# thelovelab/DESeq2

Measured on AMD Instinct MI355X. Metric: genes/sec for DESeq() disp+beta+Wald fit, 50k x 500 x p=4 (throughput of steps pipelined two deep; one call at a time: one_call_at_a_time), higher is better.
Workload: dtype f64; 1 GPU; BASELINE configs[2]: 50k genes x 500 samples, ~batch+condition (p=4), Wald; 50000 non-zero genes in total, sharded over 1 GPU(s) in the contiguous ranges of R/parallel.R:10; inputs resident in HBM in R layout (int32 counts, f64 nf matrix; the fused chain reads the size factors as the m-vector the matrix was built from); genes_total=50000, genes_this_gpu=50000, samples=500, p=4, test=Wald, parallelism=gene-shard x1, chain=fused device-driven (dsq_deseq_dev), steps_overlap=step k enqueued while step k-1's results are copied and post-processed

## Files before the change

### deseq2_amd/csrc/ctx.hip

```cpp
#include "../../include/deseq2_mi355x.h"
#include "dsq_internal.hpp"

#include <cstdarg>
#include <cstdio>
#include <cstdlib>
#include <cstring>
#include <map>
#include <memory>
#include <mutex>
#include <vector>

namespace dsq {

thread_local char g_err[512] = "";
std::mutex g_mu;

int capi_fail(int code, const char *fmt, ...) {
    va_list ap;
    va_start(ap, fmt);
    vsnprintf(g_err, sizeof g_err, fmt, ap);
    va_end(ap);
    return code;
}

int env_int(const char *name, int dflt) {
    const char *v = getenv(name);
    return (v && *v) ? atoi(v) : dflt;
}

const Tuning &tuning() {
    static Tuning t = {env_int("DSQ_BETA_WAVES", 4), env_int("DSQ_BETA_STAGE", -1), env_int("DSQ_BETA_BPC", 0),
                       env_int("DSQ_BETA_LDS_KB", 160),
                       env_int("DSQ_DISP_WAVES", 4), env_int("DSQ_DISP_STAGE", -1), env_int("DSQ_DISP_BPC", 0),
                       env_int("DSQ_DISP_LDS_KB", 160), env_int("DSQ_ABLATE", 0), env_int("DSQ_FORCE_ITERS", 0),
                       env_int("DSQ_DISP_XLDS", 1), env_int("DSQ_BETA_XLDS", 1), env_int("DSQ_DYNAMIC", 1),
                       env_int("DSQ_BETA_CELLS", 1), env_int("DSQ_DISP_CELL_MINP", DSQ_DISP_CELL_MINP),
                       env_int("DSQ_OVERLAP", 1), env_int("DSQ_LPT", 1),
                       env_int("DSQ_LPT_MAXN", 16384), env_int("DSQ_LPT_KEY2", 0)};
    return t;
}

int device_cu_count() {
    static int cached[kMaxDevices];
    int dev = 0;
    if (hipGetDevice(&dev) != hipSuccess || dev < 0 || dev >= kMaxDevices) return 256;
    if (cached[dev] == 0) {
        int v = 0;
        if (hipDeviceGetAttribute(&v, hipDeviceAttributeMultiprocessorCount, dev) != hipSuccess || v <= 0) v = 256;
        cached[dev] = v;
    }
    return cached[dev];
}

// ... 202 lines not shown
```

### deseq2_amd/csrc/dsq_internal.hpp

```cpp
#pragma once
#include <hip/hip_runtime.h>
#include <stdint.h>
#include <functional>
#include <mutex>
#include <string.h>

namespace dsq {

struct DispKernelParams {
    int n, m, p;
    long ld;
    const int32_t *y;
    const double *mu_hat;
    const double *weights;
    const double *x;
    const double *log_alpha_in;
    const double *prior_mean;
    double prior_sigmasq, min_log_alpha, kappa_0, tol, weightThreshold;
    int maxit, usePrior, useWeights, useCR;
    double *log_alpha;
    int32_t *iter, *iter_accept;
    double *last_change, *initial_lp, *initial_dlp, *last_lp, *last_dlp, *last_d2lp;
    const double *grid;
    int ngrid;
// ... 26 lines not shown
    int maxit, useQR, useWeights;
    double *beta_mat, *beta_var_mat, *iter, *hat_diagonals, *contrast_num, *contrast_denom, *deviance;
    double *mu_out;
    double *scratch;
    double *cscratch;
    int ablate, force_iters;
    int xlds;
    int *work_counter;
    const int32_t *rows;
    const int32_t *n_dev;
    int rows_few;
    const int32_t *cell_perm, *cell_start;
    int ncell;
    double *kconst_out;
    int p_true;
};

struct PrefitKernelParams {
    int n, m, p;
    long ld;
    const int32_t *y;
    const double *nf;
    int nf_is_vector;
    const double *weights;
    int useWeights;
    const double *q, *a, *r;
    double *baseMean, *baseVar, *roughDisp, *beta_init;
    int32_t *allZero;
    const int32_t *rows;
    const int32_t *n_dev;
// ... 56 lines not shown
struct CooksKernelParams {
    int n, m, p;
    long ld;
    const int32_t *y;
    const double *nf;
    int nf_is_vector;
    const double *mu, *H;
    const int32_t *perm;
    const int32_t *cell_start;
    const int32_t *in3;
    int ncell, any3;
    int sortcap;
    double *cooks, *maxCooks, *robustDisp;
    const int32_t *rows;
    const int32_t *n_dev;
};

struct ReplaceKernelParams {
    int n, m;
    long ld;
    const int32_t *y;
    const double *nf;
    int nf_is_vector;
    const double *cooks;
    double cutoff, trim;
    const int32_t *replaceable;
    int sortcap;
    int32_t *newCounts, *replace;
    const int32_t *rows;
    const int32_t *n_dev;
};

struct SizeFactorKernelParams {
    int n, m;
    const void *y;
    long y_si, y_sj;
    const double *nm;
    long nm_si, nm_sj;
    const double *geoMeans;
    const int32_t *control;
    int type;
    int stabilize;
    double *sf;
    double *lgm_out;
    double *nf_out;
// ... 113 lines not shown
template <int P> hipError_t launch_fit_beta_p(const BetaKernelParams &kp, hipStream_t st);
template <int P> hipError_t launch_optim_p(const OptimKernelParams &kp, hipStream_t st);
template <int P> void fit_beta_scratch_doubles(int n, int m, int use_weights, size_t *slab, size_t *cscr);

struct Tuning {
    int beta_waves, beta_stage, beta_bpc, beta_lds_kb;
    int disp_waves, disp_stage, disp_bpc, disp_lds_kb;
    int ablate, force_iters;
    int disp_xlds, beta_xlds;
    int dynamic;
    int beta_cells;
    int disp_cell_minp;
    int overlap;
    int lpt, lpt_maxn;
    int lpt_key2;
};
const Tuning &tuning();

hipError_t launch_transpose_r_to_gm_f64(const double *src, double *dst, int n, int m, long ld, hipStream_t st);
hipError_t launch_transpose_r_to_gm_i32(const int32_t *src, int32_t *dst, int n, int m, long ld, hipStream_t st);
hipError_t launch_counts_f64_to_gm_i32(const double *src, int32_t *dst, int n, int m, long ld, int32_t *bad, hipStream_t st);
hipError_t launch_transpose_gm_to_r_f64(const double *src, double *dst, int n, int m, long ld, hipStream_t st);
hipError_t launch_transpose_gm_to_r_i32(const int32_t *src, int32_t *dst, int n, int m, long ld, hipStream_t st);
hipError_t launch_test_math(int op, const double *a, const double *b, const double *c, double *out, long n, hipStream_t st);

constexpr int kMaxDevices = 64;
int device_cu_count();
#define DSQ_CACHE_PER_DEVICE(a, b)                                                        \
    do {                                                                                  \
        static thread_local int cache_dev_ = -1;                                          \
// ... 10 lines not shown
        if (e_ != hipSuccess)                                                                    \
            return capi_fail(e_ == hipErrorOutOfMemory ? DSQ_ERR_NOMEM : DSQ_ERR_DEVICE, "%s: %s", #expr, \
                             hipGetErrorString(e_));                                             \
    } while (0)
int env_int(const char *name, int dflt);
extern std::mutex g_mu;
void capi_latch_stream(hipStream_t s);
int capi_ws_get(int slot, size_t bytes, void **out);
int capi_upload_table(int slot, const void *src, size_t bytes, hipStream_t st, void **dev_out);
int capi_check_device();
int capi_upload_cells(const int32_t *labels, int m, int slot, hipStream_t st, const int32_t **perm_dev,
                      const int32_t **start_dev);
hipError_t launch_fit_beta_rolled(const BetaKernelParams &kp, hipStream_t st);
void fit_beta_rolled_scratch_doubles(int n, int m, int p, int useW, size_t *slab, size_t *cscr);
hipError_t dispatch_fit_beta(int p, const BetaKernelParams &kp, hipStream_t st, bool *ok);
void dispatch_beta_scratch(int p, int n, int m, int useW, size_t *slab, size_t *cscr);
hipError_t dispatch_fit_disp(int p, const DispKernelParams &kp, hipStream_t st, bool grid, bool *ok);
bool fit_disp_rolled_applies(const DispKernelParams &kp, int *p_true);
hipError_t dispatch_optim_rows(int p, const OptimKernelParams &kp, hipStream_t st, bool *ok);
void capi_prof_begin(const char *name, int n, hipStream_t st);
void capi_prof_end(hipStream_t st);
bool capi_prof_on();
int capi_side_stream(hipStream_t *side, hipEvent_t *fork_ev, hipEvent_t *join_ev);
int capi_host_sharded(size_t n, const std::function<int(size_t, size_t, hipStream_t, int, int)> &f, int max_shards);
int capi_host_shards(size_t n);
int stage_h2d(void *dev, const void *host, size_t e, size_t n_total, size_t lo, size_t cnt, size_t cols, hipStream_t st);
int stage_d2h(void *host, const void *dev, size_t e, size_t n_total, size_t lo, size_t cnt, size_t cols, hipStream_t st);
void stage_prefault(void *host, size_t bytes);
void stage_prefault_finish();
struct PrefaultScope { ~PrefaultScope() { stage_prefault_finish(); } };
// ... 7 lines not shown
```

### deseq2_amd/csrc/fit_beta.hip

```cpp
#ifndef DSQ_BETA_WIDE_MIN
#define DSQ_BETA_WIDE_MIN 10
#endif
#define DSQ_WIDE_MIN DSQ_BETA_WIDE_MIN
#include "dsq_internal.hpp"
#include <cstdio>
#include <cstdlib>
#include "dsq_math.hpp"
#include "dsq_wave.hpp"
#include "../../include/dsq_arith_spec.h"
#include "fit_beta_common.hpp"
#include "dsq_prof.hpp"

namespace dsq {

template <int P>
struct SymNB { static constexpr int value = P * (P + 1) / 2; };

#define DSQ_BETA_ARENA_MIN DSQ_WIDE_MIN
#if DSQ_P >= DSQ_BETA_ARENA_MIN
#define DSQ_BWORK(T, name) T &name = *reinterpret_cast<T *>(arena + arena_off); arena_off += (int)((sizeof(T) + 7) / 8)
#define DSQ_BMARK(name) const int name = arena_off
#define DSQ_BRESET(name) arena_off = name
#define DSQ_UNROLL_Q _Pragma("unroll")
#else
// ... 668 lines not shown
#endif

__host__ __device__ static inline size_t beta_cell_int_doubles(int m) { return (((size_t)DSQ_CMAX + 2 + m + 3) / 4) * 2; }
__host__ __device__ static inline size_t beta_cell_wave_doubles(int m, bool use_w) {
    (void)m; (void)use_w;
    return (4 + 16) * (size_t)DSQ_CMAX;
}
static_assert((4 + 16) * DSQ_CMAX >= kIrlsTab / 2 + 2 * kIrlsTab, "the constants pass borrows the wave's cell slab + park area");

#ifdef DSQ_WIDE_PROF
__device__ unsigned long long betac_prof[DSQ_PROF_SLOTS];
#define DSQ_CPROF(slot) do { const unsigned long long t1_ = clock64(); pacc_k[slot] += t1_ - pt0_k; pt0_k = t1_; } while (0)
#else
#define DSQ_CPROF(slot)
#endif
template <int P, bool USE_W>
__global__ void __launch_bounds__(256, DSQ_BETA_CELL_MINW) fit_beta_cell_kernel(BetaKernelParams kp) {
    extern __shared__ __attribute__((aligned(16))) double smem[];
    const int lane = threadIdx.x & 63;
    const int wave = threadIdx.x >> 6;
    const int waves = blockDim.x >> 6;
    const int m = kp.m;
    const int C = kp.ncell;
    const int Mrows = C + P;
    const int nwork = DSQ_NWORK(kp);
    if (blockIdx.x * waves >= nwork) return;
    double *xcs = smem;
    int32_t *starts = reinterpret_cast<int32_t *>(smem + (size_t)DSQ_CMAX * P);
    int32_t *pc = starts + DSQ_CMAX + 2;
    const size_t lnf_doubles = kp.nf_is_vector ? (size_t)m : 0;
// ... 322 lines not shown
                    for (int k = 1; k < P; k++) eta = __builtin_fma(xcs[cl * P + k], beta[k], eta);
                    double h = 0.0;
#pragma unroll
                    for (int i1 = 0; i1 < P; i1++) {
                        const double x1 = xcs[cl * P + i1];
#pragma unroll
                        for (int i2 = 0; i2 < P; i2++) h += x1 * (xcs[cl * P + i2] * lane_read(Gic[i2], i1));
                    }
                    if (lane < C) {
                        slab[4 * lane] = expl;
                        slab[4 * lane + 2] = dexp(eta);
                        slab[4 * lane + 3] = h;
                    }
                }
                wave_lds_sync();
                for (int k = lane; k < m; k += 64) {
                    const int pk = pc[k];
                    const int j = pk & 0x3ffffff, c = pk >> 26;
                    const double nf = nfg[j];
                    if (kp.hat_diagonals) {
                        const double mu = __builtin_fmax(nf * slab[4 * c], minmu);
                        const double rcp = 1.0 / (1.0 + alpha * mu);
                        double wv;
                        if constexpr (USE_W) wv = mu * (wg[j] * rcp);
                        else wv = mu * rcp;
                        kp.hat_diagonals[(size_t)g * kp.ld + j] = wv * slab[4 * c + 3];
                    }
                    if (kp.mu_out) {
                        double v = nf * slab[4 * c + 2];
                        if (kp.mu_floor > 0.0) v = __builtin_fmax(v, kp.mu_floor);
                        kp.mu_out[(size_t)g * kp.ld + j] = v;
                    }
                }
            }
            DSQ_CPROF(6);
            double Tc[P], Sgc[P];
            lane_mat_mul<P>(Gic, Gc, Tc);
            lane_mat_mul<P>(Tc, Gic, Sgc);
            double cn = 0.0;
#pragma unroll
            for (int c = 0; c < P; c++) cn = __builtin_fma(kp.contrast[c], beta[c], cn);
            double rr = 0.0;
#pragma unroll
            for (int a = 0; a < P; a++) rr = __builtin_fma(kp.contrast[a], Sgc[a], rr);
            double cd = 0.0;
#pragma unroll
            for (int b = 0; b < P; b++) cd = __builtin_fma(lane_read(rr, b), kp.contrast[b], cd);
// ... 36 lines not shown
            wave_lds_sync();
            if (lane < C) {
                double eta = xcs[lane * P] * beta[0];
#pragma unroll
                for (int k = 1; k < P; k++) eta = __builtin_fma(xcs[lane * P + k], beta[k], eta);
                double h = 0.0;
#pragma unroll
                for (int i1 = 0; i1 < P; i1++)
#pragma unroll
                    for (int i2 = 0; i2 < P; i2++) h += xcs[lane * P + i1] * (xcs[lane * P + i2] * Gi[i2][i1]);
                slab[4 * lane] = expl;
                slab[4 * lane + 2] = dexp(eta);
                slab[4 * lane + 3] = h;
            }
            wave_lds_sync();
            for (int k = lane; k < m; k += 64) {
                const int pk = pc[k];
                const int j = pk & 0x3ffffff, c = pk >> 26;
                const double nf = nfg[j];
                if (kp.hat_diagonals) {
                    const double mu = __builtin_fmax(nf * slab[4 * c], minmu);
                    const double rcp = 1.0 / (1.0 + alpha * mu);
                    double wv;
                    if constexpr (USE_W) wv = mu * (wg[j] * rcp);
                    else wv = mu * rcp;
                    kp.hat_diagonals[(size_t)g * kp.ld + j] = wv * slab[4 * c + 3];
                }
                if (kp.mu_out) {
                    double v = nf * slab[4 * c + 2];
                    if (kp.mu_floor > 0.0) v = __builtin_fmax(v, kp.mu_floor);
                    kp.mu_out[(size_t)g * kp.ld + j] = v;
                }
            }
        }
        DSQ_CPROF(6);
        double T[P][P], Sg[P][P];
        mat_mul<P>(Gi, G, T);
        mat_mul<P>(T, Gi, Sg);
        double cn = 0.0;
#pragma unroll
        for (int c = 0; c < P; c++) cn = __builtin_fma(contrast[c], beta[c], cn);
        double cd = 0.0;
#pragma unroll
        for (int b = 0; b < P; b++) {
            double rr = 0.0;
#pragma unroll
            for (int a = 0; a < P; a++) rr = __builtin_fma(contrast[a], Sg[a][b], rr);
// ... 377 lines not shown
#else
    int waves, grid, xlds;
    bool stage;
    size_t lds;
    beta_geometry<DSQ_P>(n, m, useW != 0, &waves, &stage, &xlds, &grid, &lds);
    *slab = stage ? 0 : (size_t)grid * waves * (size_t)m * kSlabVecs;
    *cscr = 0;
    if (DSQ_P >= rolled_minp()) {
        size_t s2 = 0, c2 = 0;
        fit_beta_rolled_scratch_doubles(n, m, DSQ_P, useW, &s2, &c2);
        if (s2 > *slab) *slab = s2;
    }
#endif
}

template <>
hipError_t launch_fit_beta_p<DSQ_P>(const BetaKernelParams &kp0, hipStream_t st) {
    if constexpr (DSQ_P <= DSQ_SPEC_BETA_CELL_MAXP)
        if (kp0.ncell > 0 && kp0.ncell <= DSQ_CMAX && kp0.ncell + DSQ_P <= 64) return launch_beta_cells<DSQ_P>(kp0, st);
#if DSQ_P >= DSQ_BETA_ROLLED_MIN
    return launch_fit_beta_rolled(kp0, st);
#else
    if (DSQ_P >= rolled_minp()) return launch_fit_beta_rolled(kp0, st);
    int waves, grid, xlds;
    bool stage;
    size_t lds;
    int qr = 0;
    beta_geometry<DSQ_P>(kp0.n, kp0.m, kp0.useWeights != 0, &waves, &stage, &xlds, &grid, &lds,
                         kp0.useQR != 0 && kp0.maxit > 0, &qr);
    BetaKernelParams kp = kp0;
    kp.xlds = xlds;
    if (kp.rows_few && grid > device_cu_count()) grid = device_cu_count();
    constexpr int kQr = (DSQ_P >= DSQ_BETA_QRROWS_MIN) ? 1 : 0, kQreg = (DSQ_P >= DSQ_BETA_QRREG_MIN) ? 2 : 0;
    constexpr int kQreg2 = (DSQ_P >= DSQ_BETA_QRREG_MIN && DSQ_P <= DSQ_BETA_QRREG2_MAXP) ? 3 : 0;
// ... 32 lines not shown
```

### deseq2_amd/csrc/outlier.hip

```cpp
#include "dsq_internal.hpp"
#include "dsq_math.hpp"
#include "dsq_wave.hpp"
#include <type_traits>

namespace dsq {

DSQ_DEV void wave_sort(double *b, int n2, int lane) {
    wave_lds_sync();
    for (int k = 2; k <= n2; k <<= 1) {
        for (int j = k >> 1; j > 0; j >>= 1) {
            for (int t = lane; t < (n2 >> 1); t += 64) {
                int lo = ((t & ~(j - 1)) << 1) | (t & (j - 1));
                int hi = lo | j;
                bool asc = (lo & k) == 0;
                double a = b[lo], c = b[hi];
                if ((a > c) == asc) { b[lo] = c; b[hi] = a; }
            }
            wave_lds_sync();
        }
    }
}

DSQ_DEV void wave_merge_bitonic(double *b, int n2, int lane) {
    wave_lds_sync();
// ... 35 lines not shown

static constexpr int kOutlierBatch = 4;

__global__ void __launch_bounds__(256) cooks_kernel(CooksKernelParams kp) {
    extern __shared__ double smem[];
    const int lane = threadIdx.x & 63;
    const int wave = threadIdx.x >> 6;
    const int waves = blockDim.x >> 6;
    const int m = kp.m;
    double *cn = smem + (size_t)wave * (m + kp.sortcap);
    double *buf = cn + m;
    const double inf = __builtin_inf();
    const int nwork = DSQ_NWORK(kp);
    for (int wi = blockIdx.x * waves + wave; wi < nwork; wi += gridDim.x * waves) {
        const int g = DSQ_GENE(kp, wi);
        const int32_t *yg = kp.y + (size_t)g * kp.ld;
        const double *nfg = kp.nf_is_vector ? kp.nf : kp.nf + (size_t)g * kp.ld;
        double acc = 0.0;
        {
            int32_t yb[kOutlierBatch];
            double nb[kOutlierBatch];
            sweep_batched<kOutlierBatch>(m, lane, [&](int j, int b) { yb[b] = yg[j]; nb[b] = nfg[j]; },
                                         [&](int j, int b) {
                                             const double v = (double)yb[b] / nb[b];
                                             cn[j] = v;
                                             acc += v;
                                         });
        }
        const double mean_all = wave_allreduce(acc) / (double)m;
        double v;
// ... 101 lines not shown
    }
}

__global__ void __launch_bounds__(256) replace_kernel(ReplaceKernelParams kp) {
    extern __shared__ double smem[];
    const int lane = threadIdx.x & 63;
    const int wave = threadIdx.x >> 6;
    const int waves = blockDim.x >> 6;
    const int m = kp.m;
    double *buf = smem + (size_t)wave * kp.sortcap;
    const double inf = __builtin_inf();
    const int n2 = pow2_at_least(m);
    const int nwork = DSQ_NWORK(kp);
    for (int wi = blockIdx.x * waves + wave; wi < nwork; wi += gridDim.x * waves) {
        const int g = DSQ_GENE(kp, wi);
        const int32_t *yg = kp.y + (size_t)g * kp.ld;
        const double *nfg = kp.nf_is_vector ? kp.nf : kp.nf + (size_t)g * kp.ld;
        const double *ckg = kp.cooks + (size_t)g * kp.ld;
        int any = 0;
        {
            double cb[kOutlierBatch];
            sweep_batched<kOutlierBatch>(m, lane, [&](int j, int b) { cb[b] = ckg[j]; },
                                         [&](int, int b) { if (cb[b] > kp.cutoff) any = 1; });
        }
        any = __any(any);
        int32_t *og = kp.newCounts + (size_t)g * kp.ld;
        if (!any) {
            int32_t yb[kOutlierBatch];
            sweep_batched<kOutlierBatch>(m, lane, [&](int j, int b) { yb[b] = yg[j]; }, [&](int j, int b) { og[j] = yb[b]; });
        } else {
// ... 19 lines not shown

template <typename KP, typename F>
static hipError_t launch_outlier(F fn, const KP &kp, size_t doubles_per_wave, hipStream_t st, bool *ok) {
    int waves = outlier_waves(doubles_per_wave);
    *ok = waves > 0;
    if (!*ok) return hipSuccess;
    size_t lds = (size_t)waves * doubles_per_wave * 8;
    if (lds > 64 * 1024) {
        hipError_t e = hipFuncSetAttribute((const void *)fn, hipFuncAttributeMaxDynamicSharedMemorySize, (int)lds);
        if (e != hipSuccess) return e;
    }
    int blocks = (kp.n + waves - 1) / waves;
    int per_cu = (int)((160 * 1024) / (lds ? lds : 1));
    if (per_cu > 8) per_cu = 8;
    if (per_cu < 1) per_cu = 1;
    int cap = device_cu_count() * per_cu;
    if (blocks > cap) blocks = cap;
    if (blocks < 1) blocks = 1;
    hipLaunchKernelGGL(fn, dim3(blocks), dim3(64 * waves), lds, st, kp);
    return hipGetLastError();
}

hipError_t launch_cooks(const CooksKernelParams &kp0, hipStream_t st, bool *ok) {
    CooksKernelParams kp = kp0;
    if (kp.sortcap < 64) kp.sortcap = 64;
    return launch_outlier(cooks_kernel, kp, (size_t)kp.m + kp.sortcap, st, ok);
}

hipError_t launch_replace(const ReplaceKernelParams &kp, hipStream_t st, bool *ok) {
    return launch_outlier(replace_kernel, kp, (size_t)kp.sortcap, st, ok);
}
// ... 3 lines not shown
```

### deseq2_amd/csrc/pipeline.hip

```cpp
#include "capi.hpp"
#include "dsq_math.hpp"
#include "dsq_wave.hpp"

#include <algorithm>
#include <cstdio>
#include <cstdlib>
#include <cstring>
#include <vector>

namespace dsq {

DSQ_DEV double np_min(double a, double b) { return (a != a || b != b) ? a + b : (a < b ? a : b); }
DSQ_DEV double np_max(double a, double b) { return (a != a || b != b) ? a + b : (a > b ? a : b); }

struct Rows {
    const int32_t *rows;
    const int32_t *n_dev;
    int n;
};
DSQ_DEV int rows_count(const Rows &r) { return r.n_dev ? *r.n_dev : r.n; }
DSQ_DEV int rows_gene(const Rows &r, int i) { return r.rows ? r.rows[i] : i; }

__global__ void __launch_bounds__(1024) compact_kernel(int mode, int n, int32_t *allZero, const int32_t *force_zero,
                                                       const double *mean_in, const double *disp_in, double thresh,
// ... 206 lines not shown
                const double z = q.beta[(size_t)g + (size_t)q.n * c] / q.betaSE[(size_t)g + (size_t)q.n * c];
                q.stat[(size_t)g + (size_t)q.n * c] = z;
                q.pvalue[(size_t)g + (size_t)q.n * c] = dpnorm_upper2(z);
            }
        }
    }
}

__global__ void list_kernel(Rows rw, const int32_t *flag, int want, int32_t *rows_out, int32_t *count) {
    const int i = blockIdx.x * blockDim.x + threadIdx.x;
    if (i >= rows_count(rw)) return;
    const int g = rows_gene(rw, i);
    if ((flag[g] != 0) == (want != 0)) rows_out[atomicAdd(count, 1)] = g;
}

struct NaRowsParams {
    Rows rw;
    int n, p;
    const int32_t *allZero, *n_refit;
    double *beta, *betaSE, *stat, *pvalue, *betaIter, *logLike, *logLikeReduced, *maxCooks;
    int32_t *betaConv;
};
__global__ void na_rows_kernel(NaRowsParams q) {
    const int i = blockIdx.x * blockDim.x + threadIdx.x;
    if (i >= rows_count(q.rw) || *q.n_refit <= 0) return;
    const int g = rows_gene(q.rw, i);
    if (!q.allZero[g]) return;
    const double nan = dnan();
    for (int c = 0; c < q.p; c++) {
        q.beta[(size_t)g + (size_t)q.n * c] = nan;
// ... 145 lines not shown
    const int32_t *red_cell_perm, *red_cell_start;
    int red_ncell;
    int32_t *cells_dev;
    void *trend_ws, *sel_ws;
    int pkp, pmax;
    int next_counter;
    const int32_t *cell_perm, *cell_start;
    int ncell;
    const char *tag;
    double t_tol, t_minmu, ge_floor;
    int t_maxit, t_useQR;
    hipStream_t side;
    hipEvent_t ev_fork, ev_join;
    bool overlap, forked, ll_pending;
    LogLikeKernelParams ll;
    int any3, maxcell, all_replaceable;
};

enum { CNT_NZ = DSQ_ST_N_NONZERO, CNT_GRID1 = DSQ_ST_N_GRID_GENEEST, CNT_TREND = DSQ_ST_N_TREND, CNT_GRID2 = DSQ_ST_N_GRID_MAP,
       CNT_OPT1 = DSQ_ST_N_OPTIM_GENEEST, CNT_OPT2 = DSQ_ST_N_OPTIM_TEST, CNT_REP = DSQ_ST_N_REPLACE, CNT_REFIT = DSQ_ST_N_REFIT,
       CNT_GRID1R = DSQ_ST_N_GRID_GENEEST_REFIT, CNT_GRID2R = DSQ_ST_N_GRID_MAP_REFIT, CNT_OPT1R = DSQ_ST_N_OPTIM_GENEEST_REFIT,
       CNT_OPT2R = DSQ_ST_N_OPTIM_TEST_REFIT, CNT_OPT3 = 14, CNT_OPT3R = 15, CNT_N = DSQ_ST_COUNT };
static_assert(DSQ_ST_N_OPTIM_TEST_REFIT < 14 && DSQ_ST_COUNT == 16, "status block layout");

static int *next_work_counter(Pipe &P) {
    int *c = P.work_counters + (P.next_counter % 60);
    P.next_counter++;
    return c;
}

// ... 43 lines not shown
    int ncell;
    int p_true;
};
static DesignSel design_of(const Pipe &P, int which) {
    const DsqDeseqArgs *a = P.a;
    DesignSel d;
    if (which == DES_REDUCED) d = {P.red_x_k, P.red_binit, P.red_lam, P.red_pk, P.red_cell_perm, P.red_cell_start, P.red_ncell, a->p_red};
    else if (which == DES_PRIOR) d = {P.pri_x_k, a->prior_expanded ? P.red_binit : P.beta_init, P.lam_prior, P.pri_pk,
                                      P.cell_perm, P.cell_start, P.ncell, a->p_prior};
    else d = {P.x_k, P.beta_init, P.lam, P.pk, P.cell_perm, P.cell_start, P.ncell, P.p};
    return d;
}

static int launch_fit_beta(Pipe &P, const Rows &rw, const int32_t *y, const double *alpha, const double *weights,
                           double *mu_out, double mu_floor, double *hat, double tol, int maxit, int useQR, double minmu,
                           const char *name, int which = DES_FULL) {
    const DesignSel ds = design_of(P, which);
    BetaKernelParams kp = fit_head<BetaKernelParams>(P, rw, y, weights);
    kp.p = ds.p; kp.x = ds.x; kp.alpha_hat = alpha; kp.contrast = P.contrast;
    kp.beta_init = ds.beta_init; kp.lambda = ds.lam;
    kp.tol = tol; kp.minmu = minmu; kp.mu_floor = mu_floor; kp.maxit = maxit; kp.useQR = useQR ? 1 : 0;
    kp.beta_mat = P.beta_nat; kp.beta_var_mat = P.beta_var; kp.iter = P.beta_iter;
    kp.contrast_num = P.cnum; kp.contrast_denom = P.cden; kp.deviance = P.dev;
    kp.hat_diagonals = hat; kp.mu_out = mu_out;
    kp.kconst_out = P.kconst;
    kp.scratch = P.scratch; kp.cscratch = P.cscratch;
    kp.work_counter = next_work_counter(P);
    kp.rows_few = rows_few(P, rw);
    kp.cell_perm = ds.cperm; kp.cell_start = ds.cstart; kp.ncell = ds.ncell;
    kp.p_true = ds.p_true;
    bool ok = false;
    char nm[32];
    snprintf(nm, sizeof nm, "%s%s", name, P.tag);
// ... 234 lines not shown
    DSQ_HIP(hipGetLastError());
    return DSQ_OK;
}

hipError_t launch_loglike_side(const LogLikeKernelParams &kp, hipStream_t st);
hipError_t launch_xim_flagged(const double *nf, int n, int m, long ld, const int32_t *want_a, const int32_t *want_b, double *scratch_m,
                              double *out, hipStream_t st);
static int join_side(Pipe &P) {
    if (!P.forked) return DSQ_OK;
    P.forked = false;
    DSQ_HIP(hipEventRecord(P.ev_join, P.side));
    DSQ_HIP(hipStreamWaitEvent(P.st, P.ev_join, 0));
    return DSQ_OK;
}

static int launch_pending_ll(Pipe &P, bool beside) {
    if (!P.ll_pending) return DSQ_OK;
    P.ll_pending = false;
    if (beside) {
        DSQ_HIP(hipEventRecord(P.ev_fork, P.st));
        DSQ_HIP(hipStreamWaitEvent(P.side, P.ev_fork, 0));
        DSQ_HIP(launch_loglike_side(P.ll, P.side));
        P.forked = true;
    } else {
        DSQ_HIP(launch_loglike(P.ll, P.st));
    }
    return DSQ_OK;
}

static int test_fit(Pipe &P, const Rows &rw, const int32_t *y, double *mu_out, double *hat, int cnt_optim) {
    const DsqDeseqArgs *a = P.a;
    const DsqDeseqOut *o = P.o;
    if (a->betaPrior) return mle_fit(P, rw, y, mu_out, hat);
    const bool by_mean = tuning().lpt_key2 == 1;
    int rc = launch_fit_beta(P, by_mean ? lpt_rows(P, rw, nullptr, o->baseMean, 1) : (a->linearMu ? rw : lpt_rows(P, rw, nullptr, P.beta_iter)),
                             y, o->dispersion, a->weights_norm, mu_out, 0.0, hat,
                             P.t_tol, P.t_maxit, P.t_useQR, P.t_minmu, "fit_beta");
    if (rc) return rc;
    LogLikeKernelParams lk = loglike_params(P, rw, y, mu_out, o->logLike);
    if (P.overlap && !P.tag[0]) {
        P.ll = lk;
        P.ll.skip = o->optim_test;
        P.ll_pending = true;
    } else {
        capi_prof_begin(P.tag[0] ? "nbinom_loglike:refit" : "nbinom_loglike", P.n, P.st);
        DSQ_HIP(launch_loglike(lk, P.st));
        capi_prof_end(P.st);
    }
    rc = beta_post_optim(P, rw, y, DES_FULL, (a->test == 0) ? 1 : 0, cnt_optim, mu_out);
    if (rc) return rc;
    if (a->test == 1 && a->x_red) {
        bool ok = false;
        capi_prof_begin(P.tag[0] ? "prefit_reduced:refit" : "prefit_reduced", P.n, P.st);
// ... 144 lines not shown
        !o->dispersion || !o->dispIter || !o->dispOutlier || !o->beta || !o->betaSE || !o->betaConv || !o->betaIter ||
        !o->logLike || !o->maxCooks || !o->replace || !o->optim_geneest || !o->optim_test || !o->mu_hat || !o->mu || !o->H ||
        !o->cooks || !o->replaceCounts || !o->status || !o->scalars)
        return capi_fail(DSQ_ERR_ARG, "NULL output");
    if (a->test == 0 && (!o->stat || !o->pvalue)) return capi_fail(DSQ_ERR_ARG, "Wald test needs stat / pvalue outputs");
    if (a->test == 1 && !o->logLikeReduced) return capi_fail(DSQ_ERR_ARG, "LRT needs logLikeReduced");
    if ((a->phases & (DSQ_PH_OUTLIERS | DSQ_PH_OUTLIERS_DETECT | DSQ_PH_OUTLIERS_REFIT | DSQ_PH_FINISH)) && (!a->cell_of || !a->replaceable || a->ncell < 1)) return capi_fail(DSQ_ERR_ARG, "outlier phase needs cell_of / replaceable");
    return DSQ_OK;
}

static int bind(Pipe &P, const DsqDeseqArgs *a, const DsqDeseqOut *o, hipStream_t st) {
    P.a = a; P.o = o; P.st = st; P.tag = "";
    P.t_tol = a->betaTol; P.t_maxit = a->betaMaxit; P.t_useQR = a->useQR; P.t_minmu = a->minmu; P.ge_floor = a->minmu;
    P.overlap = tuning().overlap && !capi_prof_on() && !a->betaPrior && (a->phases & DSQ_PH_MAP_TEST) && (a->phases & DSQ_PH_OUTLIERS);
    if (P.overlap && capi_side_stream(&P.side, &P.ev_fork, &P.ev_join) != DSQ_OK) P.overlap = false;
    const int n = P.n = a->n, m = P.m = a->m;
    P.p = a->p; P.ld = a->ld;
    P.maxDisp = m > 10 ? (double)m : 10.0;
    P.min_log_alpha = a->min_log_alpha;
    P.pk = kern_width(a->p);
    P.pkp = a->betaPrior ? kern_width(a->p_prior) : 0;
    P.pmax = P.pkp > P.pk ? P.pkp : P.pk;
    const int nt_cap = a->n_trend > n ? a->n_trend : n;
    const size_t need = workspace_table(P, n, P.pmax, nt_cap, nullptr);
    if (!a->workspace || a->workspace_bytes < (int64_t)need)
        return capi_fail(DSQ_ERR_ARG, "workspace of %lld bytes, dsq_deseq_workspace_bytes() asks for %zu", (long long)a->workspace_bytes, need);
    workspace_table(P, n, P.pmax, nt_cap, (double *)a->workspace);
    P.contrast = P.lam + P.pmax; P.lam_prior = P.contrast + P.pmax; P.xim_dev = P.lam + 3 * (size_t)P.pmax; P.xim_cur = P.xim_dev;
    P.counters = o->status;
    size_t slab_d = 0, cscr_d = 0;
// ... 178 lines not shown
    }
    int rc = map_est(P, nz, a->y, o->mu_hat, CNT_GRID2);
    if (rc) return rc;
    if ((rc = test_fit(P, nz, a->y, o->mu, o->H, CNT_OPT2))) return rc;
    const bool z = *counters_zeroed = (a->phases & (DSQ_PH_OUTLIERS | DSQ_PH_OUTLIERS_DETECT)) && !((a->phases & DSQ_PH_PRIOR) && a->betaPrior);
    hipLaunchKernelGGL(na_assay_rows_kernel, ew_grid(P.n), dim3(256), 0, P.st, P.n, P.m, P.ld, (const int32_t *)o->allZero, o->mu, o->H,
                       z ? P.counters + CNT_REP : (int32_t *)nullptr, z ? (int)(CNT_N - CNT_REP) : 0);
    return DSQ_OK;
}

static int phase_prior(Pipe &P, const Rows &nz) {
    DSQ_HIP(hipMemsetAsync(P.counters + CNT_OPT2, 0, sizeof(int32_t), P.st));
    return prior_fit(P, nz, P.a->y, CNT_OPT2);
}

static int phase_outlier_detect(Pipe &P, const Rows &nz, const OutlierMeta &M, bool counters_zeroed) {
    const DsqDeseqArgs *a = P.a;
    const DsqDeseqOut *o = P.o;
    const int n = P.n, m = P.m;
    hipStream_t st = P.st;
    if (!counters_zeroed) DSQ_HIP(hipMemsetAsync(P.counters + CNT_REP, 0, (CNT_N - CNT_REP) * sizeof(int32_t), st));
    CooksKernelParams ck;
    memset(&ck, 0, sizeof ck);
    ck.n = n; ck.m = m; ck.p = P.p; ck.ld = P.ld; ck.y = a->y; ck.nf = a->nf; ck.nf_is_vector = a->nf_is_vector;
    ck.mu = o->mu; ck.H = o->H; ck.perm = M.dperm; ck.cell_start = M.dstart; ck.in3 = M.din3; ck.ncell = a->ncell; ck.any3 = M.any3;
    int cap = 2; while (cap < (M.any3 ? M.maxcell : m)) cap <<= 1;
    ck.sortcap = cap;
    ck.cooks = o->cooks; ck.maxCooks = o->maxCooks; ck.robustDisp = P.robustDisp;
    ck.rows = nz.rows; ck.n_dev = nz.n_dev;
    bool ok = true;
    capi_prof_begin("cooks_distance", n, st);
    DSQ_HIP(launch_cooks(ck, st, &ok));
    capi_prof_end(st);
    if (!ok) return capi_fail(DSQ_ERR_UNSUPPORTED, "m=%d samples: a gene row plus its sort buffer exceeds the 160 KiB LDS", m);
    hipLaunchKernelGGL(na_assay_rows_kernel, ew_grid(n), dim3(256), 0, st, n, m, P.ld, (const int32_t *)o->allZero, o->cooks,
                       (double *)nullptr);
    if (!a->do_replace) return DSQ_OK;
    ReplaceKernelParams rk;
    memset(&rk, 0, sizeof rk);
    rk.n = n; rk.m = m; rk.ld = P.ld; rk.y = a->y; rk.nf = a->nf; rk.nf_is_vector = a->nf_is_vector;
    rk.cooks = o->cooks; rk.cutoff = a->cooksCutoff; rk.trim = a->trim; rk.replaceable = M.drepl;
    int cap2 = 2; while (cap2 < m) cap2 <<= 1;
    rk.sortcap = cap2;
    rk.newCounts = o->replaceCounts; rk.replace = o->replace;
    rk.rows = nz.rows; rk.n_dev = nz.n_dev;
    capi_prof_begin("replace_outliers", n, st);
    DSQ_HIP(launch_replace(rk, st, &ok));
    capi_prof_end(st);
    if (!ok) return capi_fail(DSQ_ERR_UNSUPPORTED, "m=%d samples: the sort buffer exceeds the 160 KiB LDS", m);
    hipLaunchKernelGGL(list_kernel, ew_grid(n), dim3(256), 0, st, nz, (const int32_t *)o->replace, 1, P.rows_rep, P.counters + CNT_REP);
    const Rows rep = {P.rows_rep, P.counters + CNT_REP, n};
    const int rc = launch_prefit_rows(P, rep, o->replaceCounts);
    if (rc) return rc;
    hipLaunchKernelGGL(list_kernel, ew_grid(n), dim3(256), 0, st, rep, (const int32_t *)o->allZero, 0, P.rows_refit, P.counters + CNT_REFIT);
    return DSQ_OK;
}

static void refit_defaults(Pipe &P) {
    P.tag = ":refit";
    P.t_tol = 1e-8; P.t_maxit = 100; P.t_useQR = 1; P.t_minmu = 0.5; P.ge_floor = 0.5;
}

static int phase_outlier_refit(Pipe &P, const Rows &nz, const OutlierMeta &M) {
    const DsqDeseqArgs *a = P.a;
    const DsqDeseqOut *o = P.o;
    const Rows rep = {P.rows_rep, P.counters + CNT_REP, P.n};
    const Rows rf = {P.rows_refit, P.counters + CNT_REFIT, P.n};
    int rc;
    if ((rc = launch_pending_ll(P, true))) return rc;
    refit_defaults(P);
    if (!a->nf_is_vector) {
        double *b;
        if ((rc = xim_scratch(P, &b))) return rc;
        DSQ_HIP(launch_xim_flagged(a->nf, P.n, P.m, P.ld, o->replace, o->allZero, b, P.xim_dev + 1, P.st));
        P.xim_cur = P.xim_dev + 1;
    }
    if ((rc = gene_est(P, rf, o->replaceCounts, o->mu_hat, CNT_GRID1R, CNT_OPT1R, o->optim_geneest))) return rc;
    if ((rc = map_est(P, rf, o->replaceCounts, o->mu_hat, CNT_GRID2R))) return rc;
    if ((rc = join_side(P))) return rc;
    if ((rc = test_fit(P, rf, o->replaceCounts, o->mu_hat, nullptr, CNT_OPT2R))) return rc;
    if (a->betaPrior && (rc = prior_fit(P, rf, o->replaceCounts, CNT_OPT2R))) return rc;
    return a->defer_finish ? DSQ_OK : outlier_finish(P, nz, rep, M, P.counters + CNT_REFIT);
}

static int run_chain(const DsqDeseqArgs *a, const DsqDeseqOut *o, hipStream_t st, Pipe &P) {
    int rc = check_args(a, o);
    if (rc || (rc = capi_check_device()) || (rc = bind(P, a, o, st)) || (rc = launch_init_fills(P)) || (rc = prepare_designs(P))) return rc;
    const Rows nz = {P.rows_nz, P.counters + CNT_NZ, P.n};
    const int ph = a->phases;
    if ((ph & DSQ_PH_GENE_EST) && (rc = phase_gene_est(P, nz))) return rc;
    if ((ph & DSQ_PH_TREND) && (rc = phase_trend(P))) return rc;
    bool counters_zeroed = false;
    if ((ph & DSQ_PH_MAP_TEST) && (rc = phase_map_test(P, nz, &counters_zeroed))) return rc;
    if ((ph & DSQ_PH_PRIOR) && a->betaPrior && (rc = phase_prior(P, nz))) return rc;
    const bool detect = (ph & (DSQ_PH_OUTLIERS | DSQ_PH_OUTLIERS_DETECT)) != 0, refit = (ph & (DSQ_PH_OUTLIERS | DSQ_PH_OUTLIERS_REFIT)) != 0;
    OutlierMeta M;
    if ((detect || refit || ((ph & DSQ_PH_FINISH) && a->do_replace)) && (rc = outlier_meta(a, P.m, st, &M))) return rc;
    if (detect && (rc = phase_outlier_detect(P, nz, M, counters_zeroed))) return rc;
    if (refit && a->do_replace && (rc = phase_outlier_refit(P, nz, M))) return rc;
    if ((ph & DSQ_PH_FINISH) && a->do_replace)
        return outlier_finish(P, nz, Rows{P.rows_rep, P.counters + CNT_REP, P.n}, M, a->n_refit_global ? a->n_refit_global : P.counters + CNT_REFIT);
    return DSQ_OK;
}

static int run(const DsqDeseqArgs *a, const DsqDeseqOut *o, hipStream_t st) {
    Pipe P;
    memset(&P, 0, sizeof P);
    const int rc = run_chain(a, o, st, P);
    const int rl = rc ? DSQ_OK : launch_pending_ll(P, false);
    const int rj = join_side(P);
    return rc ? rc : (rl ? rl : rj);
}

int pipeline_run(const DsqDeseqArgs *a, const DsqDeseqOut *o, hipStream_t st) { return run(a, o, st); }
// ... 16 lines not shown
```

Before: 5.493 million genes/s.

## Flag Cook's outlier candidates during beta fit and process them first

The Wald beta-fit cell kernel now evaluates a conservative bound on each sample's Cook's distance and sets a per-gene candidate flag. The outlier phase lists these candidates, together with optimizer-flagged genes, and runs Cook's distance, replacement and refit for them on the main stream. Cook's and replacement for all other genes run on the side stream alongside the log-likelihood kernel, using a reduced grid. The intent is to take the full-width Cook's/replace pass off the critical path ahead of the refit. The cost is an extra per-sample bound check in the fit kernel and more complex stream and event ordering.

```diff
diff --git a/deseq2_amd/csrc/ctx.hip b/deseq2_amd/csrc/ctx.hip
--- a/deseq2_amd/csrc/ctx.hip
+++ b/deseq2_amd/csrc/ctx.hip
@@ -36,7 +36,7 @@
                        env_int("DSQ_DISP_XLDS", 1), env_int("DSQ_BETA_XLDS", 1), env_int("DSQ_DYNAMIC", 1),
                        env_int("DSQ_BETA_CELLS", 1), env_int("DSQ_DISP_CELL_MINP", DSQ_DISP_CELL_MINP),
                        env_int("DSQ_OVERLAP", 1), env_int("DSQ_LPT", 1),
-                       env_int("DSQ_LPT_MAXN", 16384), env_int("DSQ_LPT_KEY2", 0)};
+                       env_int("DSQ_LPT_MAXN", 16384), env_int("DSQ_LPT_KEY2", 0), env_int("DSQ_OUTLIER_FIRST", 1)};
     return t;
 }
 
diff --git a/deseq2_amd/csrc/dsq_internal.hpp b/deseq2_amd/csrc/dsq_internal.hpp
--- a/deseq2_amd/csrc/dsq_internal.hpp
+++ b/deseq2_amd/csrc/dsq_internal.hpp
@@ -64,6 +64,8 @@
     int ncell;
     double *kconst_out;
     int p_true;
+    int32_t *cand_flag;
+    double cand_cutoff, cand_p;
 };
 
 struct PrefitKernelParams {
@@ -150,6 +152,9 @@
     double *cooks, *maxCooks, *robustDisp;
     const int32_t *rows;
     const int32_t *n_dev;
+    const int32_t *skip;
+    int rows_few;
+    int beside;
 };
 
 struct ReplaceKernelParams {
@@ -165,6 +170,8 @@
     int32_t *newCounts, *replace;
     const int32_t *rows;
     const int32_t *n_dev;
+    const int32_t *skip;
+    int rows_few, beside;
 };
 
 struct SizeFactorKernelParams {
@@ -308,6 +315,7 @@
     int overlap;
     int lpt, lpt_maxn;
     int lpt_key2;
+    int outlier_first;
 };
 const Tuning &tuning();
 
@@ -348,6 +356,7 @@
 hipError_t launch_fit_beta_rolled(const BetaKernelParams &kp, hipStream_t st);
 void fit_beta_rolled_scratch_doubles(int n, int m, int p, int useW, size_t *slab, size_t *cscr);
 hipError_t dispatch_fit_beta(int p, const BetaKernelParams &kp, hipStream_t st, bool *ok);
+static inline bool fit_beta_on_cells(int p, int ncell) { return p <= 32  && ncell > 0 && ncell <= DSQ_CMAX && ncell + p <= 64; }
 void dispatch_beta_scratch(int p, int n, int m, int useW, size_t *slab, size_t *cscr);
 hipError_t dispatch_fit_disp(int p, const DispKernelParams &kp, hipStream_t st, bool grid, bool *ok);
 bool fit_disp_rolled_applies(const DispKernelParams &kp, int *p_true);
diff --git a/deseq2_amd/csrc/fit_beta.hip b/deseq2_amd/csrc/fit_beta.hip
--- a/deseq2_amd/csrc/fit_beta.hip
+++ b/deseq2_amd/csrc/fit_beta.hip
@@ -706,6 +706,24 @@
 #else
 #define DSQ_CPROF(slot)
 #endif
+DSQ_DEV bool cooks_can_exceed(double y, double mu, double h, double p, double cutoff) {
+    const double V = mu + 0.04 * (mu * mu);
+    const double d = y - mu;
+#ifdef DSQ_CAND_DIVFREE
+    const double omh = 1.0 - h;
+    const double L = (d * d) * h;
+    const double R = ((cutoff * p) * V) * (omh * omh);
+    const bool below = (L * (1.0 + 0x1p-40) <= R) && (R >= 1e-280) && (R < __builtin_inf()) && (h >= 0.0) && (h < 1.0) &&
+                       (cutoff * p >= 1e-100);
+    return !below;
+#else
+    const double pr = (d * d) / V;
+    const double omh = 1.0 - h;
+    const double B = pr / p * h / (omh * omh);
+    return !(B <= cutoff) || !(h >= 0.0);
+#endif
+}
+
 template <int P, bool USE_W>
 __global__ void __launch_bounds__(256, DSQ_BETA_CELL_MINW) fit_beta_cell_kernel(BetaKernelParams kp) {
     extern __shared__ __attribute__((aligned(16))) double smem[];
@@ -1058,23 +1076,32 @@
                     }
                 }
                 wave_lds_sync();
+                int cand = 0;
                 for (int k = lane; k < m; k += 64) {
                     const int pk = pc[k];
                     const int j = pk & 0x3ffffff, c = pk >> 26;
                     const double nf = nfg[j];
+                    double hj = 0.0, mj = 0.0;
                     if (kp.hat_diagonals) {
                         const double mu = __builtin_fmax(nf * slab[4 * c], minmu);
                         const double rcp = 1.0 / (1.0 + alpha * mu);
                         double wv;
                         if constexpr (USE_W) wv = mu * (wg[j] * rcp);
                         else wv = mu * rcp;
-                        kp.hat_diagonals[(size_t)g * kp.ld + j] = wv * slab[4 * c + 3];
+                        hj = wv * slab[4 * c + 3];
+                        kp.hat_diagonals[(size_t)g * kp.ld + j] = hj;
                     }
                     if (kp.mu_out) {
                         double v = nf * slab[4 * c + 2];
                         if (kp.mu_floor > 0.0) v = __builtin_fmax(v, kp.mu_floor);
                         kp.mu_out[(size_t)g * kp.ld + j] = v;
-                    }
+                        mj = v;
+                    }
+                    if (kp.cand_flag) cand |= cooks_can_exceed((double)yg[j], mj, hj, kp.cand_p, kp.cand_cutoff) ? 1 : 0;
+                }
+                if (kp.cand_flag) {
+                    const int any = __any(cand);
+                    if (lane == 0) kp.cand_flag[g] = any ? 1 : 0;
                 }
             }
             DSQ_CPROF(6);
@@ -1141,23 +1168,32 @@
                 slab[4 * lane + 3] = h;
             }
             wave_lds_sync();
+            int cand = 0;
             for (int k = lane; k < m; k += 64) {
                 const int pk = pc[k];
                 const int j = pk & 0x3ffffff, c = pk >> 26;
                 const double nf = nfg[j];
+                double hj = 0.0, mj = 0.0;
                 if (kp.hat_diagonals) {
                     const double mu = __builtin_fmax(nf * slab[4 * c], minmu);
                     const double rcp = 1.0 / (1.0 + alpha * mu);
                     double wv;
                     if constexpr (USE_W) wv = mu * (wg[j] * rcp);
                     else wv = mu * rcp;
-                    kp.hat_diagonals[(size_t)g * kp.ld + j] = wv * slab[4 * c + 3];
+                    hj = wv * slab[4 * c + 3];
+                    kp.hat_diagonals[(size_t)g * kp.ld + j] = hj;
                 }
                 if (kp.mu_out) {
                     double v = nf * slab[4 * c + 2];
                     if (kp.mu_floor > 0.0) v = __builtin_fmax(v, kp.mu_floor);
                     kp.mu_out[(size_t)g * kp.ld + j] = v;
-                }
+                    mj = v;
+                }
+                if (kp.cand_flag) cand |= cooks_can_exceed((double)yg[j], mj, hj, kp.cand_p, kp.cand_cutoff) ? 1 : 0;
+            }
+            if (kp.cand_flag) {
+                const int any = __any(cand);
+                if (lane == 0) kp.cand_flag[g] = any ? 1 : 0;
             }
         }
         DSQ_CPROF(6);
@@ -1565,10 +1601,11 @@
 #endif
 }
 
+static_assert(DSQ_SPEC_BETA_CELL_MAXP == 32, "fit_beta_on_cells (dsq_internal.hpp) states the widest cell kernel");
 template <>
 hipError_t launch_fit_beta_p<DSQ_P>(const BetaKernelParams &kp0, hipStream_t st) {
     if constexpr (DSQ_P <= DSQ_SPEC_BETA_CELL_MAXP)
-        if (kp0.ncell > 0 && kp0.ncell <= DSQ_CMAX && kp0.ncell + DSQ_P <= 64) return launch_beta_cells<DSQ_P>(kp0, st);
+        if (fit_beta_on_cells(DSQ_P, kp0.ncell)) return launch_beta_cells<DSQ_P>(kp0, st);
 #if DSQ_P >= DSQ_BETA_ROLLED_MIN
     return launch_fit_beta_rolled(kp0, st);
 #else
diff --git a/deseq2_amd/csrc/outlier.hip b/deseq2_amd/csrc/outlier.hip
--- a/deseq2_amd/csrc/outlier.hip
+++ b/deseq2_amd/csrc/outlier.hip
@@ -73,6 +73,7 @@
     const int nwork = DSQ_NWORK(kp);
     for (int wi = blockIdx.x * waves + wave; wi < nwork; wi += gridDim.x * waves) {
         const int g = DSQ_GENE(kp, wi);
+        if (kp.skip && kp.skip[g]) continue;
         const int32_t *yg = kp.y + (size_t)g * kp.ld;
         const double *nfg = kp.nf_is_vector ? kp.nf : kp.nf + (size_t)g * kp.ld;
         double acc = 0.0;
@@ -204,6 +205,7 @@
     const int nwork = DSQ_NWORK(kp);
     for (int wi = blockIdx.x * waves + wave; wi < nwork; wi += gridDim.x * waves) {
         const int g = DSQ_GENE(kp, wi);
+        if (kp.skip && kp.skip[g]) continue;
         const int32_t *yg = kp.y + (size_t)g * kp.ld;
         const double *nfg = kp.nf_is_vector ? kp.nf : kp.nf + (size_t)g * kp.ld;
         const double *ckg = kp.cooks + (size_t)g * kp.ld;
@@ -253,7 +255,20 @@
     int per_cu = (int)((160 * 1024) / (lds ? lds : 1));
     if (per_cu > 8) per_cu = 8;
     if (per_cu < 1) per_cu = 1;
-    int cap = device_cu_count() * per_cu;
+    if (kp.beside) {
+        static thread_local int occ_cache[1];
+        static thread_local size_t lds_cache[1];
+        DSQ_CACHE_PER_DEVICE(occ_cache, lds_cache);
+        if (lds_cache[0] != lds || occ_cache[0] == 0) {
+            int occ = 0;
+            if (hipOccupancyMaxActiveBlocksPerMultiprocessor(&occ, (const void *)fn, 64 * waves, lds) != hipSuccess || occ < 1) occ = per_cu;
+            occ_cache[0] = occ; lds_cache[0] = lds;
+        }
+        if (occ_cache[0] < per_cu) per_cu = occ_cache[0];
+        per_cu /= 2;
+        if (per_cu < 1) per_cu = 1;
+    }
+    int cap = device_cu_count() * (kp.rows_few ? 1 : per_cu);
     if (blocks > cap) blocks = cap;
     if (blocks < 1) blocks = 1;
     hipLaunchKernelGGL(fn, dim3(blocks), dim3(64 * waves), lds, st, kp);
diff --git a/deseq2_amd/csrc/pipeline.hip b/deseq2_amd/csrc/pipeline.hip
--- a/deseq2_amd/csrc/pipeline.hip
+++ b/deseq2_amd/csrc/pipeline.hip
@@ -244,6 +244,16 @@
     if ((flag[g] != 0) == (want != 0)) rows_out[atomicAdd(count, 1)] = g;
 }
 
+__global__ void cand_list_kernel(Rows rw, const int32_t *bound_flag, const int32_t *optim_flag, int32_t *flag_out, int32_t *rows_out,
+                                 int32_t *count) {
+    const int i = blockIdx.x * blockDim.x + threadIdx.x;
+    if (i >= rows_count(rw)) return;
+    const int g = rows_gene(rw, i);
+    const int f = (bound_flag[g] != 0 || optim_flag[g] != 0) ? 1 : 0;
+    flag_out[g] = f;
+    if (f) rows_out[atomicAdd(count, 1)] = g;
+}
+
 struct NaRowsParams {
     Rows rw;
     int n, p;
@@ -419,6 +429,7 @@
     hipEvent_t ev_fork, ev_join;
     bool overlap, forked, ll_pending;
     LogLikeKernelParams ll;
+    bool outlier_first, cand_ready, ll_event;
     int any3, maxcell, all_replaceable;
 };
 
@@ -492,9 +503,10 @@
 
 static int launch_fit_beta(Pipe &P, const Rows &rw, const int32_t *y, const double *alpha, const double *weights,
                            double *mu_out, double mu_floor, double *hat, double tol, int maxit, int useQR, double minmu,
-                           const char *name, int which = DES_FULL) {
+                           const char *name, int which = DES_FULL, bool cand = false) {
     const DesignSel ds = design_of(P, which);
     BetaKernelParams kp = fit_head<BetaKernelParams>(P, rw, y, weights);
+    if (cand) { kp.cand_flag = P.grid_flag; kp.cand_cutoff = P.a->cooksCutoff; kp.cand_p = (double)P.p; }
     kp.p = ds.p; kp.x = ds.x; kp.alpha_hat = alpha; kp.contrast = P.contrast;
     kp.beta_init = ds.beta_init; kp.lambda = ds.lam;
     kp.tol = tol; kp.minmu = minmu; kp.mu_floor = mu_floor; kp.maxit = maxit; kp.useQR = useQR ? 1 : 0;
@@ -759,14 +771,21 @@
     return DSQ_OK;
 }
 
+static int fork_side(Pipe &P) {
+    if (P.forked) return DSQ_OK;
+    DSQ_HIP(hipEventRecord(P.ev_fork, P.st));
+    DSQ_HIP(hipStreamWaitEvent(P.side, P.ev_fork, 0));
+    P.forked = true;
+    return DSQ_OK;
+}
+
 static int launch_pending_ll(Pipe &P, bool beside) {
     if (!P.ll_pending) return DSQ_OK;
     P.ll_pending = false;
     if (beside) {
-        DSQ_HIP(hipEventRecord(P.ev_fork, P.st));
-        DSQ_HIP(hipStreamWaitEvent(P.side, P.ev_fork, 0));
+        const int rc = fork_side(P);
+        if (rc) return rc;
         DSQ_HIP(launch_loglike_side(P.ll, P.side));
-        P.forked = true;
     } else {
         DSQ_HIP(launch_loglike(P.ll, P.st));
     }
@@ -778,10 +797,12 @@
     const DsqDeseqOut *o = P.o;
     if (a->betaPrior) return mle_fit(P, rw, y, mu_out, hat);
     const bool by_mean = tuning().lpt_key2 == 1;
+    const bool cand = P.outlier_first && !P.tag[0] && hat && !(a->test == 1 && a->x_red) && fit_beta_on_cells(P.pk, P.ncell);
     int rc = launch_fit_beta(P, by_mean ? lpt_rows(P, rw, nullptr, o->baseMean, 1) : (a->linearMu ? rw : lpt_rows(P, rw, nullptr, P.beta_iter)),
                              y, o->dispersion, a->weights_norm, mu_out, 0.0, hat,
-                             P.t_tol, P.t_maxit, P.t_useQR, P.t_minmu, "fit_beta");
-    if (rc) return rc;
+                             P.t_tol, P.t_maxit, P.t_useQR, P.t_minmu, "fit_beta", DES_FULL, cand);
+    if (rc) return rc;
+    if (cand) P.cand_ready = true;
     LogLikeKernelParams lk = loglike_params(P, rw, y, mu_out, o->logLike);
     if (P.overlap && !P.tag[0]) {
         P.ll = lk;
@@ -956,6 +977,7 @@
     P.t_tol = a->betaTol; P.t_maxit = a->betaMaxit; P.t_useQR = a->useQR; P.t_minmu = a->minmu; P.ge_floor = a->minmu;
     P.overlap = tuning().overlap && !capi_prof_on() && !a->betaPrior && (a->phases & DSQ_PH_MAP_TEST) && (a->phases & DSQ_PH_OUTLIERS);
     if (P.overlap && capi_side_stream(&P.side, &P.ev_fork, &P.ev_join) != DSQ_OK) P.overlap = false;
+    P.outlier_first = P.overlap && tuning().outlier_first && a->do_replace && (a->phases & DSQ_PH_GENE_EST);
     const int n = P.n = a->n, m = P.m = a->m;
     P.p = a->p; P.ld = a->ld;
     P.maxDisp = m > 10 ? (double)m : 10.0;
@@ -1164,46 +1186,101 @@
     return prior_fit(P, nz, P.a->y, CNT_OPT2);
 }
 
+static CooksKernelParams cooks_params(const Pipe &P, const OutlierMeta &M, const Rows &rw) {
+    const DsqDeseqArgs *a = P.a;
+    const DsqDeseqOut *o = P.o;
+    CooksKernelParams ck;
+    memset(&ck, 0, sizeof ck);
+    ck.n = P.n; ck.m = P.m; ck.p = P.p; ck.ld = P.ld; ck.y = a->y; ck.nf = a->nf; ck.nf_is_vector = a->nf_is_vector;
+    ck.mu = o->mu; ck.H = o->H; ck.perm = M.dperm; ck.cell_start = M.dstart; ck.in3 = M.din3; ck.ncell = a->ncell; ck.any3 = M.any3;
+    int cap = 2; while (cap < (M.any3 ? M.maxcell : P.m)) cap <<= 1;
+    ck.sortcap = cap;
+    ck.cooks = o->cooks; ck.maxCooks = o->maxCooks; ck.robustDisp = P.robustDisp;
+    ck.rows = rw.rows; ck.n_dev = rw.n_dev;
+    return ck;
+}
+static ReplaceKernelParams replace_params(const Pipe &P, const OutlierMeta &M, const Rows &rw) {
+    const DsqDeseqArgs *a = P.a;
+    const DsqDeseqOut *o = P.o;
+    ReplaceKernelParams rk;
+    memset(&rk, 0, sizeof rk);
+    rk.n = P.n; rk.m = P.m; rk.ld = P.ld; rk.y = a->y; rk.nf = a->nf; rk.nf_is_vector = a->nf_is_vector;
+    rk.cooks = o->cooks; rk.cutoff = a->cooksCutoff; rk.trim = a->trim; rk.replaceable = M.drepl;
+    int cap2 = 2; while (cap2 < P.m) cap2 <<= 1;
+    rk.sortcap = cap2;
+    rk.newCounts = o->replaceCounts; rk.replace = o->replace;
+    rk.rows = rw.rows; rk.n_dev = rw.n_dev;
+    return rk;
+}
+static int launch_cooks_rows(Pipe &P, const CooksKernelParams &ck, hipStream_t st) {
+    bool ok = true;
+    capi_prof_begin("cooks_distance", P.n, st);
+    DSQ_HIP(launch_cooks(ck, st, &ok));
+    capi_prof_end(st);
+    if (!ok) return capi_fail(DSQ_ERR_UNSUPPORTED, "m=%d samples: a gene row plus its sort buffer exceeds the 160 KiB LDS", P.m);
+    return DSQ_OK;
+}
+static int launch_replace_rows(Pipe &P, const ReplaceKernelParams &rk, hipStream_t st) {
+    bool ok = true;
+    capi_prof_begin("replace_outliers", P.n, st);
+    DSQ_HIP(launch_replace(rk, st, &ok));
+    capi_prof_end(st);
+    if (!ok) return capi_fail(DSQ_ERR_UNSUPPORTED, "m=%d samples: the sort buffer exceeds the 160 KiB LDS", P.m);
+    return DSQ_OK;
+}
+
+static int list_replaced(Pipe &P, const Rows &from) {
+    const DsqDeseqOut *o = P.o;
+    hipLaunchKernelGGL(list_kernel, ew_grid(P.n), dim3(256), 0, P.st, from, (const int32_t *)o->replace, 1, P.rows_rep, P.counters + CNT_REP);
+    const Rows rep = {P.rows_rep, P.counters + CNT_REP, P.n};
+    const int rc = launch_prefit_rows(P, rep, o->replaceCounts);
+    if (rc) return rc;
+    hipLaunchKernelGGL(list_kernel, ew_grid(P.n), dim3(256), 0, P.st, rep, (const int32_t *)o->allZero, 0, P.rows_refit, P.counters + CNT_REFIT);
+    return DSQ_OK;
+}
+
 static int phase_outlier_detect(Pipe &P, const Rows &nz, const OutlierMeta &M, bool counters_zeroed) {
     const DsqDeseqArgs *a = P.a;
     const DsqDeseqOut *o = P.o;
     const int n = P.n, m = P.m;
     hipStream_t st = P.st;
     if (!counters_zeroed) DSQ_HIP(hipMemsetAsync(P.counters + CNT_REP, 0, (CNT_N - CNT_REP) * sizeof(int32_t), st));
-    CooksKernelParams ck;
-    memset(&ck, 0, sizeof ck);
-    ck.n = n; ck.m = m; ck.p = P.p; ck.ld = P.ld; ck.y = a->y; ck.nf = a->nf; ck.nf_is_vector = a->nf_is_vector;
-    ck.mu = o->mu; ck.H = o->H; ck.perm = M.dperm; ck.cell_start = M.dstart; ck.in3 = M.din3; ck.ncell = a->ncell; ck.any3 = M.any3;
-    int cap = 2; while (cap < (M.any3 ? M.maxcell : m)) cap <<= 1;
-    ck.sortcap = cap;
-    ck.cooks = o->cooks; ck.maxCooks = o->maxCooks; ck.robustDisp = P.robustDisp;
-    ck.rows = nz.rows; ck.n_dev = nz.n_dev;
-    bool ok = true;
-    capi_prof_begin("cooks_distance", n, st);
-    DSQ_HIP(launch_cooks(ck, st, &ok));
-    capi_prof_end(st);
-    if (!ok) return capi_fail(DSQ_ERR_UNSUPPORTED, "m=%d samples: a gene row plus its sort buffer exceeds the 160 KiB LDS", m);
+    int rc = launch_cooks_rows(P, cooks_params(P, M, nz), st);
+    if (rc) return rc;
     hipLaunchKernelGGL(na_assay_rows_kernel, ew_grid(n), dim3(256), 0, st, n, m, P.ld, (const int32_t *)o->allZero, o->cooks,
                        (double *)nullptr);
     if (!a->do_replace) return DSQ_OK;
-    ReplaceKernelParams rk;
-    memset(&rk, 0, sizeof rk);
-    rk.n = n; rk.m = m; rk.ld = P.ld; rk.y = a->y; rk.nf = a->nf; rk.nf_is_vector = a->nf_is_vector;
-    rk.cooks = o->cooks; rk.cutoff = a->cooksCutoff; rk.trim = a->trim; rk.replaceable = M.drepl;
-    int cap2 = 2; while (cap2 < m) cap2 <<= 1;
-    rk.sortcap = cap2;
-    rk.newCounts = o->replaceCounts; rk.replace = o->replace;
-    rk.rows = nz.rows; rk.n_dev = nz.n_dev;
-    capi_prof_begin("replace_outliers", n, st);
-    DSQ_HIP(launch_replace(rk, st, &ok));
-    capi_prof_end(st);
-    if (!ok) return capi_fail(DSQ_ERR_UNSUPPORTED, "m=%d samples: the sort buffer exceeds the 160 KiB LDS", m);
-    hipLaunchKernelGGL(list_kernel, ew_grid(n), dim3(256), 0, st, nz, (const int32_t *)o->replace, 1, P.rows_rep, P.counters + CNT_REP);
-    const Rows rep = {P.rows_rep, P.counters + CNT_REP, n};
-    const int rc = launch_prefit_rows(P, rep, o->replaceCounts);
-    if (rc) return rc;
-    hipLaunchKernelGGL(list_kernel, ew_grid(n), dim3(256), 0, st, rep, (const int32_t *)o->allZero, 0, P.rows_refit, P.counters + CNT_REFIT);
-    return DSQ_OK;
+    if ((rc = launch_replace_rows(P, replace_params(P, M, nz), st))) return rc;
+    return list_replaced(P, nz);
+}
+
+static int phase_outlier_refit(Pipe &P, const Rows &nz, const OutlierMeta &M);
+
+static int phase_outlier_first(Pipe &P, const Rows &nz, const OutlierMeta &M, bool counters_zeroed) {
+    const DsqDeseqOut *o = P.o;
+    const int n = P.n, m = P.m;
+    hipStream_t st = P.st;
+    if (!counters_zeroed) DSQ_HIP(hipMemsetAsync(P.counters + CNT_REP, 0, (CNT_N - CNT_REP) * sizeof(int32_t), st));
+    int32_t *skip = P.rows_lpt, *n_cand = next_work_counter(P);
+    if (getenv("DSQ_VERBOSE")) fprintf(stderr, "[dsq] outlier phase: candidates first (n=%d)\n", n);
+    hipLaunchKernelGGL(cand_list_kernel, ew_grid(n), dim3(256), 0, st, nz, (const int32_t *)P.grid_flag, (const int32_t *)o->optim_test,
+                       skip, P.rows_grid, n_cand);
+    hipLaunchKernelGGL(na_assay_rows_kernel, ew_grid(n), dim3(256), 0, st, n, m, P.ld, (const int32_t *)o->allZero, o->cooks,
+                       (double *)nullptr);
+    int rc;
+    if ((rc = fork_side(P)) || (rc = launch_pending_ll(P, true))) return rc;
+    DSQ_HIP(hipEventRecord(P.ev_fork, P.side));
+    P.ll_event = true;
+    CooksKernelParams ck = cooks_params(P, M, nz);
+    ReplaceKernelParams rk = replace_params(P, M, nz);
+    ck.skip = rk.skip = skip;
+    ck.beside = rk.beside = 1;
+    if ((rc = launch_cooks_rows(P, ck, P.side)) || (rc = launch_replace_rows(P, rk, P.side))) return rc;
+    const Rows cand = {P.rows_grid, n_cand, n};
+    ck = cooks_params(P, M, cand); rk = replace_params(P, M, cand);
+    ck.rows_few = rk.rows_few = 1;
+    if ((rc = launch_cooks_rows(P, ck, st)) || (rc = launch_replace_rows(P, rk, st)) || (rc = list_replaced(P, cand))) return rc;
+    return phase_outlier_refit(P, nz, M);
 }
 
 static void refit_defaults(Pipe &P) {
@@ -1227,9 +1304,13 @@
     }
     if ((rc = gene_est(P, rf, o->replaceCounts, o->mu_hat, CNT_GRID1R, CNT_OPT1R, o->optim_geneest))) return rc;
     if ((rc = map_est(P, rf, o->replaceCounts, o->mu_hat, CNT_GRID2R))) return rc;
-    if ((rc = join_side(P))) return rc;
+    if (P.ll_event) {
+        P.ll_event = false;
+        DSQ_HIP(hipStreamWaitEvent(P.st, P.ev_fork, 0));
+    } else if ((rc = join_side(P))) return rc;
     if ((rc = test_fit(P, rf, o->replaceCounts, o->mu_hat, nullptr, CNT_OPT2R))) return rc;
     if (a->betaPrior && (rc = prior_fit(P, rf, o->replaceCounts, CNT_OPT2R))) return rc;
+    if ((rc = join_side(P))) return rc;
     return a->defer_finish ? DSQ_OK : outlier_finish(P, nz, rep, M, P.counters + CNT_REFIT);
 }
 
@@ -1246,8 +1327,12 @@
     const bool detect = (ph & (DSQ_PH_OUTLIERS | DSQ_PH_OUTLIERS_DETECT)) != 0, refit = (ph & (DSQ_PH_OUTLIERS | DSQ_PH_OUTLIERS_REFIT)) != 0;
     OutlierMeta M;
     if ((detect || refit || ((ph & DSQ_PH_FINISH) && a->do_replace)) && (rc = outlier_meta(a, P.m, st, &M))) return rc;
-    if (detect && (rc = phase_outlier_detect(P, nz, M, counters_zeroed))) return rc;
-    if (refit && a->do_replace && (rc = phase_outlier_refit(P, nz, M))) return rc;
+    if ((ph & DSQ_PH_OUTLIERS) && P.cand_ready) {
+        if ((rc = phase_outlier_first(P, nz, M, counters_zeroed))) return rc;
+    } else {
+        if (detect && (rc = phase_outlier_detect(P, nz, M, counters_zeroed))) return rc;
+        if (refit && a->do_replace && (rc = phase_outlier_refit(P, nz, M))) return rc;
+    }
     if ((ph & DSQ_PH_FINISH) && a->do_replace)
         return outlier_finish(P, nz, Rows{P.rows_rep, P.counters + CNT_REP, P.n}, M, a->n_refit_global ? a->n_refit_global : P.counters + CNT_REFIT);
     return DSQ_OK;
```

Result: faster. 5.580 million genes/s (median of 6 runs) (+1.6%).
